# janisgp/go_with_the_flows

Measured on AMD Instinct MI355X. Metric: point-flow fwd+logdet Mpoints/sec (B x 2048 pts), higher is better.
Workload: dtype f32 (split-f16 x3 MFMA, fp32 accumulate); 1 GPU; configs[1] airplane generative (config_generative_modeling_airplane.yaml): K=4 flows x 33 couplings, f=37, G=128, B=64 x N=2048, inverse + sum(logvars) + mixture NLL, eval BN -- leads the line because it is the largest single-GPU config of BASELINE.json (configs[1]); the north-star shape B=32 x 2048, f=64 is also.m1; per_gpu_batch=64, components=4, couplings_per_component=33, f=37, G=128, direction=inverse, point_definition=one 3-D point through one component stack (coords + sum logvars)

## Files before the change

go_with_the_flows_amd/csrc/gwtf_film.hip:

```cpp
#include <hip/hip_runtime.h>
#include "gwtf_layout.h"
#include "../../include/gwtf.h"

namespace {

constexpr int kBTe = 16;

typedef float f32x4 __attribute__((ext_vector_type(4)));

template <int MB, int kGCH>
__global__ __launch_bounds__(MB > 4 ? 512 : 256) void film_eval_kernel(const float* __restrict__ g, const float* __restrict__ pf,
                                                        float* __restrict__ out, int B, int G, int C, int f, float eps) {
  constexpr int FP = 16 * MB;
  __shared__ __align__(16) float hb[2][16][FP + 4];
  const int c = blockIdx.x, br = blockIdx.y, b0 = blockIdx.z * kBTe;
  const int lane = threadIdx.x & 63, wave = threadIdx.x >> 6;
  const int q = lane >> 4, i16 = lane & 15;
  const GwtfPackF P(FP, G);
  const int GP = P.GP();
  const float* w = pf + ((size_t)c * 2 + br) * P.branch_size();
  const size_t FS = gwtf_film_out_size(FP);
  const bool own = wave < MB;
  const int ft = 16 * wave + i16;
  const int brow = b0 + i16;
  const float* grow = g + (size_t)(brow < B ? brow : B - 1) * G;
  const float* l0 = w + P.l0t(0) + 4 * ft;
  const float* l1 = w + P.l0t(1) + 4 * ft;
  const bool gvec = (G & 3) == 0;

  f32x4 acc[2] = {{0.f, 0.f, 0.f, 0.f}, {0.f, 0.f, 0.f, 0.f}};
  f32x4 w1[2][MB];
  if (own) {
#pragma unroll
    for (int kg = 0; kg < MB; ++kg)
#pragma unroll
      for (int which = 0; which < 2; ++which)
#pragma unroll
        for (int t = 0; t < 4; ++t) w1[which][kg][t] = w[P.l1t(which) + ((size_t)(4 * kg + q) * FP + ft) * 4 + t];
    for (int i0 = 0; i0 < GP; i0 += kGCH) {
      f32x4 a4[kGCH / 16], b4[2][kGCH / 16];
#pragma unroll
      for (int kg = 0; kg < kGCH / 16; ++kg) {
        if (i0 + 16 * kg < GP) {
          const int col = i0 + 16 * kg + 4 * q;
          if (gvec) {
            a4[kg] = *reinterpret_cast<const f32x4*>(grow + (col < G ? col : G - 4));
          } else {
#pragma unroll
            for (int t = 0; t < 4; ++t) a4[kg][t] = grow[col + t < G ? col + t : G - 1];
          }
          b4[0][kg] = *reinterpret_cast<const f32x4*>(l0 + (size_t)col * FP);
          b4[1][kg] = *reinterpret_cast<const f32x4*>(l1 + (size_t)col * FP);
        }
      }
#pragma unroll
      for (int kg = 0; kg < kGCH / 16; ++kg) {
        if (i0 + 16 * kg < GP) {
#pragma unroll
          for (int t = 0; t < 4; ++t) {
            acc[0] = __builtin_amdgcn_mfma_f32_16x16x4f32(a4[kg][t], b4[0][kg][t], acc[0], 0, 0, 0);
            acc[1] = __builtin_amdgcn_mfma_f32_16x16x4f32(a4[kg][t], b4[1][kg][t], acc[1], 0, 0, 0);
          }
        }
      }
    }
#pragma unroll
    for (int which = 0; which < 2; ++which) {
      const float sc = w[P.s(which) + ft], sh = w[P.t(which) + ft];
#pragma unroll
      for (int r = 0; r < 4; ++r) {
        const float h = fmaf(acc[which][r], sc, sh);
        hb[which][4 * q + r][ft] = h / (1.0f + expf(-h));
      }
    }
  }
  __syncthreads();
  if (!own) return;
  f32x4 o[2];
#pragma unroll
  for (int which = 0; which < 2; ++which) {
    const float bias = w[P.l1b(which) + ft];
    o[which] = f32x4{bias, bias, bias, bias};
  }
#pragma unroll
  for (int kg = 0; kg < MB; ++kg) {
    const f32x4 a0 = *reinterpret_cast<const f32x4*>(&hb[0][i16][16 * kg + 4 * q]);
    const f32x4 a1 = *reinterpret_cast<const f32x4*>(&hb[1][i16][16 * kg + 4 * q]);
#pragma unroll
    for (int t = 0; t < 4; ++t) {
      o[0] = __builtin_amdgcn_mfma_f32_16x16x4f32(a0[t], w1[0][kg][t], o[0], 0, 0, 0);
      o[1] = __builtin_amdgcn_mfma_f32_16x16x4f32(a1[t], w1[1][kg][t], o[1], 0, 0, 0);
    }
  }
  const float c1 = w[P.c1() + ft], w20 = w[P.w2() + ft], w21 = w[P.w2() + FP + ft];
  const float qnan = __builtin_bit_cast(float, 0x7fc00000u);
  const float poison = w[P.poison()];
#pragma unroll
  for (int r = 0; r < 4; ++r) {
    const int b = b0 + 4 * q + r;
    if (b < B) {
      float cv = 0.f, u0 = 0.f, u1 = 0.f;
      if (ft < f) {
        const float a = eps + expf(o[0][r]);
        cv = c1 + o[1][r] / a;
        u0 = w20 * a;
        u1 = w21 * a;
        if (gwtf_nonfinite(o[0][r]) || gwtf_nonfinite(o[1][r])) cv = u0 = u1 = qnan;
      }
      float* ob = out + ((size_t)b * C + c) * FS + (size_t)br * 3 * FP + ft;
      ob[0] = cv;
      ob[FP] = u0;
      ob[2 * FP] = u1;
      if (ft < 2) out[((size_t)b * C + c) * FS + 6 * FP + 2 * br + ft] = w[P.b2() + ft] + poison;
    }
  }
}

}

extern "C" int gwtf_film_forward(const float* g, const float* packed_film, float* film_out, int B, int G, int C, int f, float eps,
                                 void* stream) {
  if (B <= 0 || G <= 0 || C <= 0 || f <= 0 || f > GWTF_MAX_FP || !g || !packed_film || !film_out) return GWTF_E_BADARG;
  const int FP = gwtf_padded_width(f);
  hipStream_t st = (hipStream_t)stream;
  const dim3 grid(C, 2, (B + kBTe - 1) / kBTe);
  const bool many = (long)grid.x * grid.y * grid.z > 768;
#define GWTF_FILM_EVAL(MB_)                                                                                                  \
  if (many) hipLaunchKernelGGL((film_eval_kernel<MB_, 64>), grid, dim3(MB_ > 4 ? 512 : 256), 0, st, g, packed_film, film_out, B, G, C, f, eps); \
  else hipLaunchKernelGGL((film_eval_kernel<MB_, 128>), grid, dim3(MB_ > 4 ? 512 : 256), 0, st, g, packed_film, film_out, B, G, C, f, eps)
  switch (FP / 16) {
    case 1: GWTF_FILM_EVAL(1); break;
    case 2: GWTF_FILM_EVAL(2); break;
    case 3: GWTF_FILM_EVAL(3); break;
    case 4: GWTF_FILM_EVAL(4); break;
    case 5: GWTF_FILM_EVAL(5); break;
    case 6: GWTF_FILM_EVAL(6); break;
    case 7: GWTF_FILM_EVAL(7); break;
    default: GWTF_FILM_EVAL(8); break;
  }
#undef GWTF_FILM_EVAL
  return (int)hipGetLastError();
}
```

go_with_the_flows_amd/csrc/gwtf_nll.hip:

```cpp
#include <hip/hip_runtime.h>
#include <math.h>
#include "../../include/gwtf.h"

namespace {

constexpr int kMaxK = 64;
constexpr int kThreads = 256;
constexpr int kPtsPerBlock = 512;

__global__ __launch_bounds__(1024) void nll_kernel(const float* __restrict__ z, const float* __restrict__ logdet,
                                                       const float* __restrict__ mu0, const float* __restrict__ lv0,
                                                       const float* __restrict__ logits, float* __restrict__ point_lse,
                                                       float* __restrict__ nll_shape, int K, int B, int N) {
  __shared__ float s_logw[kMaxK];
  __shared__ float s_mu[kMaxK][3], s_lv[kMaxK][3], s_iv[kMaxK][3];
  __shared__ float s_part[16];
  const int b = blockIdx.y;
  const int ppb = gridDim.x == 1 ? N : kPtsPerBlock;
  if (threadIdx.x < 64) {
    float m = -INFINITY;
    for (int k = 0; k < K; ++k) m = fmaxf(m, logits[(size_t)b * K + k]);
    float s = 0.f;
    for (int k = 0; k < K; ++k) s += expf(logits[(size_t)b * K + k] - m);
    const float lse = m + logf(s);
    for (int k = threadIdx.x; k < K; k += 64) s_logw[k] = logf(expf(logits[(size_t)b * K + k])) - lse;
  }
  for (int t = threadIdx.x; t < K * 3; t += blockDim.x) {
    const int k = t / 3, d = t % 3;
    const float l = lv0[((size_t)k * B + b) * 3 + d];
    s_mu[k][d] = mu0[((size_t)k * B + b) * 3 + d];
    s_lv[k][d] = l;
    s_iv[k][d] = 1.0f / expf(l);
  }
  __syncthreads();
  const float half_log2pi3 = 0.5f * 3.0f * 1.8378770664093453f;
  float local = 0.f;
  const int n_end = min(N, (int)(blockIdx.x + 1) * ppb);
  for (int n = blockIdx.x * ppb + threadIdx.x; n < n_end; n += blockDim.x) {
    float m = -INFINITY, s = 0.f;
    bool nan_seen = false;
    for (int k = 0; k < K; ++k) {
      float qsum = 0.f;
#pragma unroll
      for (int d = 0; d < 3; ++d) {
        const size_t o = (((size_t)k * B + b) * 3 + d) * N + n;
        const float diff = z[o] - s_mu[k][d];
        qsum += (s_lv[k][d] + logdet[o]) + diff * diff * s_iv[k][d];
      }
      float lp = -0.5f * qsum - half_log2pi3 + s_logw[k];
      asm volatile("" : "+v"(lp));
      nan_seen |= (__float_as_uint(lp) & 0x7fffffffu) > 0x7f800000u;
      if (lp == -INFINITY) continue;
      if (lp > m || k == 0) {
        s = s * expf(m - lp) + 1.0f;
        m = lp;
      } else {
        s += expf(lp - m);
      }
    }
    const float lse = nan_seen ? __uint_as_float(0x7fc00000u) : m + logf(s);
    if (point_lse) point_lse[(size_t)b * N + n] = lse;
    local += lse;
  }
#pragma unroll
  for (int off = 32; off > 0; off >>= 1) local += __shfl_down(local, off);
  if ((threadIdx.x & 63) == 0) s_part[threadIdx.x >> 6] = local;
  __syncthreads();
  if (threadIdx.x == 0) {
    float t = 0.f;
    for (int w = 0; w < (int)blockDim.x / 64; ++w) t += s_part[w];
    if (gridDim.x == 1) nll_shape[b] = -t;
    else atomicAdd(&nll_shape[b], -t);
  }
}

__global__ __launch_bounds__(kThreads) void nll_bwd_kernel(const float* __restrict__ z, const float* __restrict__ logdet,
                                                           const float* __restrict__ mu0, const float* __restrict__ lv0,
                                                           const float* __restrict__ logits,
                                                           const float* __restrict__ point_lse,
                                                           const float* __restrict__ g_nll, float* __restrict__ g_z,
                                                           float* __restrict__ g_ld, float* __restrict__ g_mu0,
                                                           float* __restrict__ g_lv0, float* __restrict__ g_logits, int K,
                                                           int B, int N) {
  __shared__ float s_logw[kMaxK], s_sm[kMaxK];
  __shared__ float s_mu[kMaxK][3], s_lv[kMaxK][3], s_iv[kMaxK][3];
  __shared__ float s_acc[kMaxK][7];
  const int b = blockIdx.y;
  if (threadIdx.x < 64) {
    float m = -INFINITY;
    for (int k = 0; k < K; ++k) m = fmaxf(m, logits[(size_t)b * K + k]);
    float sden = 0.f;
    for (int k = 0; k < K; ++k) sden += expf(logits[(size_t)b * K + k] - m);
    const float lse = m + logf(sden);
    for (int k = threadIdx.x; k < K; k += 64) {
      s_logw[k] = logf(expf(logits[(size_t)b * K + k])) - lse;
      s_sm[k] = expf(logits[(size_t)b * K + k] - lse);
    }
  }
  for (int t = threadIdx.x; t < K * 3; t += blockDim.x) {
    const int k = t / 3, d = t % 3;
    const float l = lv0[((size_t)k * B + b) * 3 + d];
    s_mu[k][d] = mu0[((size_t)k * B + b) * 3 + d];
    s_lv[k][d] = l;
    s_iv[k][d] = 1.0f / expf(l);
  }
  for (int t = threadIdx.x; t < K * 7; t += blockDim.x) (&s_acc[0][0])[t] = 0.f;
  __syncthreads();
  const float half_log2pi3 = 0.5f * 3.0f * 1.8378770664093453f;
  const float gb = g_nll[b];
  const int n_end = min(N, (int)(blockIdx.x + 1) * kPtsPerBlock);
  for (int k = 0; k < K; ++k) {
    float a[7] = {0.f, 0.f, 0.f, 0.f, 0.f, 0.f, 0.f};
    for (int n = blockIdx.x * kPtsPerBlock + threadIdx.x; n < n_end; n += blockDim.x) {
      float diff[3], qsum = 0.f;
#pragma unroll
      for (int d = 0; d < 3; ++d) {
        const size_t o = (((size_t)k * B + b) * 3 + d) * N + n;
        diff[d] = z[o] - s_mu[k][d];
        qsum += (s_lv[k][d] + logdet[o]) + diff[d] * diff[d] * s_iv[k][d];
      }
      const float r = expf(-0.5f * qsum - half_log2pi3 + s_logw[k] - point_lse[(size_t)b * N + n]) * gb;
#pragma unroll
      for (int d = 0; d < 3; ++d) {
        const size_t o = (((size_t)k * B + b) * 3 + d) * N + n;
        const float w = diff[d] * s_iv[k][d];
        g_z[o] = r * w;
        g_ld[o] = 0.5f * r;
        a[d] -= r * w;
        a[3 + d] += r * (0.5f - 0.5f * diff[d] * w);
      }
      a[6] += r;
    }
#pragma unroll
    for (int i = 0; i < 7; ++i) {
#pragma unroll
      for (int off = 32; off > 0; off >>= 1) a[i] += __shfl_down(a[i], off);
    }
    if ((threadIdx.x & 63) == 0) {
#pragma unroll
      for (int i = 0; i < 7; ++i) atomicAdd(&s_acc[k][i], a[i]);
    }
  }
  __syncthreads();
  for (int t = threadIdx.x; t < K * 7; t += blockDim.x) {
    const int k = t / 7, i = t % 7;
    const float v = s_acc[k][i];
    if (i < 3) atomicAdd(&g_mu0[((size_t)k * B + b) * 3 + i], v);
    else if (i < 6) atomicAdd(&g_lv0[((size_t)k * B + b) * 3 + (i - 3)], v);
    else {
      const int pts = n_end - blockIdx.x * kPtsPerBlock;
      atomicAdd(&g_logits[(size_t)b * K + k], -v + gb * (float)pts * s_sm[k]);
    }
  }
}

}

extern "C" int gwtf_mixture_nll_backward(const float* z, const float* logdet, const float* mu0, const float* lv0,
                                         const float* logits, const float* point_lse, const float* g_nll, float* g_z,
                                         float* g_logdet, float* g_mu0, float* g_lv0, float* g_logits, int K, int B, int N,
                                         void* stream) {
  if (K <= 0 || K > kMaxK || B <= 0 || N <= 0 || !z || !logdet || !mu0 || !lv0 || !logits || !point_lse || !g_nll || !g_z ||
      !g_logdet || !g_mu0 || !g_lv0 || !g_logits)
    return GWTF_E_BADARG;
  hipStream_t st = (hipStream_t)stream;
  hipError_t e = hipMemsetAsync(g_mu0, 0, sizeof(float) * (size_t)K * B * 3, st);
  if (e == hipSuccess) e = hipMemsetAsync(g_lv0, 0, sizeof(float) * (size_t)K * B * 3, st);
  if (e == hipSuccess) e = hipMemsetAsync(g_logits, 0, sizeof(float) * (size_t)B * K, st);
  if (e != hipSuccess) return (int)e;
  const dim3 grid((N + kPtsPerBlock - 1) / kPtsPerBlock, B);
  hipLaunchKernelGGL(nll_bwd_kernel, grid, dim3(kThreads), 0, st, z, logdet, mu0, lv0, logits, point_lse, g_nll, g_z,
                     g_logdet, g_mu0, g_lv0, g_logits, K, B, N);
  return (int)hipGetLastError();
}

extern "C" int gwtf_mixture_nll(const float* z, const float* logdet, const float* mu0, const float* lv0,
                                const float* logits, float* point_lse, float* nll_shape, int K, int B, int N,
                                void* stream) {
  if (K <= 0 || K > kMaxK || B <= 0 || N <= 0 || !z || !logdet || !mu0 || !lv0 || !logits || !nll_shape)
    return GWTF_E_BADARG;
  hipStream_t st = (hipStream_t)stream;
  if (N <= 4096 && B >= 16) {
    hipLaunchKernelGGL(nll_kernel, dim3(1, B), dim3(1024), 0, st, z, logdet, mu0, lv0, logits, point_lse, nll_shape, K, B, N);
    return (int)hipGetLastError();
  }
  hipError_t e = hipMemsetAsync(nll_shape, 0, sizeof(float) * (size_t)B, st);
  if (e != hipSuccess) return (int)e;
  const dim3 grid((N + kPtsPerBlock - 1) / kPtsPerBlock, B);
  hipLaunchKernelGGL(nll_kernel, grid, dim3(kThreads), 0, st, z, logdet, mu0, lv0, logits, point_lse, nll_shape, K, B, N);
  return (int)hipGetLastError();
}
```

Baseline: 1076 Mpoints/s.

## Software-pipeline FiLM GEMM loads and batch mixture NLL loads across components

The FiLM kernel gains a fast path, used when G is a multiple of 4 and GP divides the chunk size. It prefetches the next chunk of g and layer-0 weights while issuing MFMAs on the current chunk, and parameter loads are hoisted ahead of the GEMM. Launches now use 64*MB threads, which drops the idle waves that previously existed for small MB. The NLL kernel issues the first group of component loads before the shared-memory setup and the __syncthreads. It then processes two points per thread, loading four components at a time to raise memory-level parallelism. The cost is higher register pressure and more complex control flow.

```diff
diff --git a/go_with_the_flows_amd/csrc/gwtf_film.hip b/go_with_the_flows_amd/csrc/gwtf_film.hip
--- a/go_with_the_flows_amd/csrc/gwtf_film.hip
+++ b/go_with_the_flows_amd/csrc/gwtf_film.hip
@@ -8,10 +8,29 @@
 
 typedef float f32x4 __attribute__((ext_vector_type(4)));
 
-template <int MB, int kGCH>
+template <int NKG>
+struct FilmChunk {
+  f32x4 a[NKG], b[2][NKG];
+  __device__ __forceinline__ void load(int kg, const float* grow, const float* l0, const float* l1, int i0, int q, int G, int FP) {
+    const int col = i0 + 16 * kg + 4 * q;
+    a[kg] = *reinterpret_cast<const f32x4*>(grow + (col < G ? col : G - 4));
+    b[0][kg] = *reinterpret_cast<const f32x4*>(l0 + (size_t)col * FP);
+    b[1][kg] = *reinterpret_cast<const f32x4*>(l1 + (size_t)col * FP);
+  }
+  __device__ __forceinline__ void mfma(int kg, f32x4 (&acc)[2]) const {
+#pragma unroll
+    for (int t = 0; t < 4; ++t) {
+      acc[0] = __builtin_amdgcn_mfma_f32_16x16x4f32(a[kg][t], b[0][kg][t], acc[0], 0, 0, 0);
+      acc[1] = __builtin_amdgcn_mfma_f32_16x16x4f32(a[kg][t], b[1][kg][t], acc[1], 0, 0, 0);
+    }
+  }
+};
+
+template <int MB, int kGCH, bool kFast>
 __global__ __launch_bounds__(MB > 4 ? 512 : 256) void film_eval_kernel(const float* __restrict__ g, const float* __restrict__ pf,
                                                         float* __restrict__ out, int B, int G, int C, int f, float eps) {
   constexpr int FP = 16 * MB;
+  constexpr int NKG = kGCH / 16;
   __shared__ __align__(16) float hb[2][16][FP + 4];
   const int c = blockIdx.x, br = blockIdx.y, b0 = blockIdx.z * kBTe;
   const int lane = threadIdx.x & 63, wave = threadIdx.x >> 6;
@@ -20,68 +39,84 @@
   const int GP = P.GP();
   const float* w = pf + ((size_t)c * 2 + br) * P.branch_size();
   const size_t FS = gwtf_film_out_size(FP);
-  const bool own = wave < MB;
   const int ft = 16 * wave + i16;
   const int brow = b0 + i16;
   const float* grow = g + (size_t)(brow < B ? brow : B - 1) * G;
   const float* l0 = w + P.l0t(0) + 4 * ft;
   const float* l1 = w + P.l0t(1) + 4 * ft;
-  const bool gvec = (G & 3) == 0;
 
   f32x4 acc[2] = {{0.f, 0.f, 0.f, 0.f}, {0.f, 0.f, 0.f, 0.f}};
   f32x4 w1[2][MB];
-  if (own) {
+  float sc[2], sh[2], bias[2], c1, w20, w21, poison, b2v;
+  FilmChunk<NKG> ch;
+  if constexpr (kFast) {
 #pragma unroll
-    for (int kg = 0; kg < MB; ++kg)
+    for (int kg = 0; kg < NKG; ++kg) ch.load(kg, grow, l0, l1, 0, q, G, FP);
+  }
 #pragma unroll
-      for (int which = 0; which < 2; ++which)
+  for (int kg = 0; kg < MB; ++kg)
 #pragma unroll
-        for (int t = 0; t < 4; ++t) w1[which][kg][t] = w[P.l1t(which) + ((size_t)(4 * kg + q) * FP + ft) * 4 + t];
+    for (int which = 0; which < 2; ++which)
+#pragma unroll
+      for (int t = 0; t < 4; ++t) w1[which][kg][t] = w[P.l1t(which) + ((size_t)(4 * kg + q) * FP + ft) * 4 + t];
+#pragma unroll
+  for (int which = 0; which < 2; ++which) {
+    sc[which] = w[P.s(which) + ft];
+    sh[which] = w[P.t(which) + ft];
+    bias[which] = w[P.l1b(which) + ft];
+  }
+  c1 = w[P.c1() + ft];
+  w20 = w[P.w2() + ft];
+  w21 = w[P.w2() + FP + ft];
+  poison = w[P.poison()];
+  b2v = w[P.b2() + (ft & 1)];
+  if constexpr (kFast) {
+    int i0 = 0;
+    for (; i0 + kGCH < GP; i0 += kGCH) {
+#pragma unroll
+      for (int kg = 0; kg < NKG; ++kg) {
+        ch.mfma(kg, acc);
+        ch.load(kg, grow, l0, l1, i0 + kGCH, q, G, FP);
+        __builtin_amdgcn_sched_barrier(0);
+      }
+    }
+#pragma unroll
+    for (int kg = 0; kg < NKG; ++kg) ch.mfma(kg, acc);
+  } else {
+    const bool gvec = (G & 3) == 0;
     for (int i0 = 0; i0 < GP; i0 += kGCH) {
-      f32x4 a4[kGCH / 16], b4[2][kGCH / 16];
 #pragma unroll
-      for (int kg = 0; kg < kGCH / 16; ++kg) {
+      for (int kg = 0; kg < NKG; ++kg) {
         if (i0 + 16 * kg < GP) {
-          const int col = i0 + 16 * kg + 4 * q;
           if (gvec) {
-            a4[kg] = *reinterpret_cast<const f32x4*>(grow + (col < G ? col : G - 4));
+            ch.load(kg, grow, l0, l1, i0, q, G, FP);
           } else {
+            const int col = i0 + 16 * kg + 4 * q;
 #pragma unroll
-            for (int t = 0; t < 4; ++t) a4[kg][t] = grow[col + t < G ? col + t : G - 1];
+            for (int t = 0; t < 4; ++t) ch.a[kg][t] = grow[col + t < G ? col + t : G - 1];
+            ch.b[0][kg] = *reinterpret_cast<const f32x4*>(l0 + (size_t)col * FP);
+            ch.b[1][kg] = *reinterpret_cast<const f32x4*>(l1 + (size_t)col * FP);
           }
-          b4[0][kg] = *reinterpret_cast<const f32x4*>(l0 + (size_t)col * FP);
-          b4[1][kg] = *reinterpret_cast<const f32x4*>(l1 + (size_t)col * FP);
         }
       }
 #pragma unroll
-      for (int kg = 0; kg < kGCH / 16; ++kg) {
-        if (i0 + 16 * kg < GP) {
-#pragma unroll
-          for (int t = 0; t < 4; ++t) {
-            acc[0] = __builtin_amdgcn_mfma_f32_16x16x4f32(a4[kg][t], b4[0][kg][t], acc[0], 0, 0, 0);
-            acc[1] = __builtin_amdgcn_mfma_f32_16x16x4f32(a4[kg][t], b4[1][kg][t], acc[1], 0, 0, 0);
-          }
-        }
-      }
-    }
-#pragma unroll
-    for (int which = 0; which < 2; ++which) {
-      const float sc = w[P.s(which) + ft], sh = w[P.t(which) + ft];
-#pragma unroll
-      for (int r = 0; r < 4; ++r) {
-        const float h = fmaf(acc[which][r], sc, sh);
-        hb[which][4 * q + r][ft] = h / (1.0f + expf(-h));
+      for (int kg = 0; kg < NKG; ++kg) {
+        if (i0 + 16 * kg < GP) ch.mfma(kg, acc);
       }
     }
   }
+#pragma unroll
+  for (int which = 0; which < 2; ++which) {
+#pragma unroll
+    for (int r = 0; r < 4; ++r) {
+      const float h = fmaf(acc[which][r], sc[which], sh[which]);
+      hb[which][4 * q + r][ft] = h / (1.0f + expf(-h));
+    }
+  }
   __syncthreads();
-  if (!own) return;
   f32x4 o[2];
 #pragma unroll
-  for (int which = 0; which < 2; ++which) {
-    const float bias = w[P.l1b(which) + ft];
-    o[which] = f32x4{bias, bias, bias, bias};
-  }
+  for (int which = 0; which < 2; ++which) o[which] = f32x4{bias[which], bias[which], bias[which], bias[which]};
 #pragma unroll
   for (int kg = 0; kg < MB; ++kg) {
     const f32x4 a0 = *reinterpret_cast<const f32x4*>(&hb[0][i16][16 * kg + 4 * q]);
@@ -92,9 +127,8 @@
       o[1] = __builtin_amdgcn_mfma_f32_16x16x4f32(a1[t], w1[1][kg][t], o[1], 0, 0, 0);
     }
   }
-  const float c1 = w[P.c1() + ft], w20 = w[P.w2() + ft], w21 = w[P.w2() + FP + ft];
   const float qnan = __builtin_bit_cast(float, 0x7fc00000u);
-  const float poison = w[P.poison()];
+  const float b2p = b2v + poison;
 #pragma unroll
   for (int r = 0; r < 4; ++r) {
     const int b = b0 + 4 * q + r;
@@ -111,7 +145,7 @@
       ob[0] = cv;
       ob[FP] = u0;
       ob[2 * FP] = u1;
-      if (ft < 2) out[((size_t)b * C + c) * FS + 6 * FP + 2 * br + ft] = w[P.b2() + ft] + poison;
+      if (ft < 2) out[((size_t)b * C + c) * FS + 6 * FP + 2 * br + ft] = b2p;
     }
   }
 }
@@ -125,9 +159,18 @@
   hipStream_t st = (hipStream_t)stream;
   const dim3 grid(C, 2, (B + kBTe - 1) / kBTe);
   const bool many = (long)grid.x * grid.y * grid.z > 768;
-#define GWTF_FILM_EVAL(MB_)                                                                                                  \
-  if (many) hipLaunchKernelGGL((film_eval_kernel<MB_, 64>), grid, dim3(MB_ > 4 ? 512 : 256), 0, st, g, packed_film, film_out, B, G, C, f, eps); \
-  else hipLaunchKernelGGL((film_eval_kernel<MB_, 128>), grid, dim3(MB_ > 4 ? 512 : 256), 0, st, g, packed_film, film_out, B, G, C, f, eps)
+  const int GP = GwtfPackF(FP, G).GP();
+  const bool fast64 = (G & 3) == 0 && GP % 64 == 0, fast128 = (G & 3) == 0 && GP % 128 == 0;
+#define GWTF_FILM_EVAL_(MB_, CH_, FAST_)                                                                                        \
+  hipLaunchKernelGGL((film_eval_kernel<MB_, CH_, FAST_>), grid, dim3(64 * MB_), 0, st, g, packed_film, film_out, B, G, C, f, eps)
+#define GWTF_FILM_EVAL(MB_)                                                                                                    \
+  if (many) {                                                                                                                  \
+    if (fast64) GWTF_FILM_EVAL_(MB_, 64, true);                                                                                \
+    else GWTF_FILM_EVAL_(MB_, 64, false);                                                                                      \
+  } else {                                                                                                                     \
+    if (fast128) GWTF_FILM_EVAL_(MB_, 128, true);                                                                              \
+    else GWTF_FILM_EVAL_(MB_, 128, false);                                                                                     \
+  }
   switch (FP / 16) {
     case 1: GWTF_FILM_EVAL(1); break;
     case 2: GWTF_FILM_EVAL(2); break;
@@ -139,5 +182,6 @@
     default: GWTF_FILM_EVAL(8); break;
   }
 #undef GWTF_FILM_EVAL
+#undef GWTF_FILM_EVAL_
   return (int)hipGetLastError();
 }
diff --git a/go_with_the_flows_amd/csrc/gwtf_nll.hip b/go_with_the_flows_amd/csrc/gwtf_nll.hip
--- a/go_with_the_flows_amd/csrc/gwtf_nll.hip
+++ b/go_with_the_flows_amd/csrc/gwtf_nll.hip
@@ -7,6 +7,61 @@
 constexpr int kMaxK = 64;
 constexpr int kThreads = 256;
 constexpr int kPtsPerBlock = 512;
+
+constexpr int kPass = 2;
+
+struct NllPoint {
+  float m, s;
+  bool nan_seen;
+};
+
+template <int NB>
+__device__ __forceinline__ void nll_load(const float* __restrict__ z, const float* __restrict__ logdet, int kb, int B, int b, int N,
+                                         const unsigned (&np)[kPass], float (&zz)[kPass][4][3], float (&ld)[kPass][4][3]) {
+  asm volatile("" : "+s"(kb));
+#pragma unroll
+  for (int j = 0; j < NB; ++j)
+#pragma unroll
+    for (int d = 0; d < 3; ++d) {
+      const size_t row = (((size_t)(kb + j) * B + b) * 3 + d) * N;
+#pragma unroll
+      for (int p = 0; p < kPass; ++p) {
+        zz[p][j][d] = (z + row)[np[p]];
+        ld[p][j][d] = (logdet + row)[np[p]];
+      }
+    }
+  __builtin_amdgcn_sched_barrier(0);
+}
+
+template <int NB>
+__device__ __forceinline__ void nll_accumulate(const float (*s_mu)[3], const float (*s_lv)[3], const float (*s_iv)[3], const float* s_logw,
+                                               int kb, const float (&zz)[kPass][4][3], const float (&ld)[kPass][4][3],
+                                               NllPoint (&pt)[kPass]) {
+  const float half_log2pi3 = 0.5f * 3.0f * 1.8378770664093453f;
+#pragma unroll
+  for (int p = 0; p < kPass; ++p)
+#pragma unroll
+    for (int j = 0; j < NB; ++j) {
+      const int k = kb + j;
+      float qsum = 0.f;
+#pragma unroll
+      for (int d = 0; d < 3; ++d) {
+        const float diff = zz[p][j][d] - s_mu[k][d];
+        qsum += (s_lv[k][d] + ld[p][j][d]) + diff * diff * s_iv[k][d];
+      }
+      float lp = -0.5f * qsum - half_log2pi3 + s_logw[k];
+      asm volatile("" : "+v"(lp));
+      pt[p].nan_seen |= (__float_as_uint(lp) & 0x7fffffffu) > 0x7f800000u;
+      if (!(lp == -INFINITY)) {
+        if (lp > pt[p].m || k == 0) {
+          pt[p].s = pt[p].s * expf(pt[p].m - lp) + 1.0f;
+          pt[p].m = lp;
+        } else {
+          pt[p].s += expf(lp - pt[p].m);
+        }
+      }
+    }
+}
 
 __global__ __launch_bounds__(1024) void nll_kernel(const float* __restrict__ z, const float* __restrict__ logdet,
                                                        const float* __restrict__ mu0, const float* __restrict__ lv0,
@@ -17,6 +72,19 @@
   __shared__ float s_part[16];
   const int b = blockIdx.y;
   const int ppb = gridDim.x == 1 ? N : kPtsPerBlock;
+  const int n_end = min(N, (int)(blockIdx.x + 1) * ppb);
+  const int n_first = blockIdx.x * ppb + threadIdx.x;
+  unsigned np[kPass];
+  float zz[kPass][4][3], ld[kPass][4][3];
+  bool ahead = K >= 4;
+  if (ahead) {
+#pragma unroll
+    for (int p = 0; p < kPass; ++p) {
+      const int n = n_first + p * (int)blockDim.x;
+      np[p] = n < n_end ? n : min(n_first, n_end - 1);
+    }
+    nll_load<4>(z, logdet, 0, B, b, N, np, zz, ld);
+  }
   if (threadIdx.x < 64) {
     float m = -INFINITY;
     for (int k = 0; k < K; ++k) m = fmaxf(m, logits[(size_t)b * K + k]);
@@ -33,34 +101,44 @@
     s_iv[k][d] = 1.0f / expf(l);
   }
   __syncthreads();
-  const float half_log2pi3 = 0.5f * 3.0f * 1.8378770664093453f;
   float local = 0.f;
-  const int n_end = min(N, (int)(blockIdx.x + 1) * ppb);
-  for (int n = blockIdx.x * ppb + threadIdx.x; n < n_end; n += blockDim.x) {
-    float m = -INFINITY, s = 0.f;
-    bool nan_seen = false;
-    for (int k = 0; k < K; ++k) {
-      float qsum = 0.f;
-#pragma unroll
-      for (int d = 0; d < 3; ++d) {
-        const size_t o = (((size_t)k * B + b) * 3 + d) * N + n;
-        const float diff = z[o] - s_mu[k][d];
-        qsum += (s_lv[k][d] + logdet[o]) + diff * diff * s_iv[k][d];
-      }
-      float lp = -0.5f * qsum - half_log2pi3 + s_logw[k];
-      asm volatile("" : "+v"(lp));
-      nan_seen |= (__float_as_uint(lp) & 0x7fffffffu) > 0x7f800000u;
-      if (lp == -INFINITY) continue;
-      if (lp > m || k == 0) {
-        s = s * expf(m - lp) + 1.0f;
-        m = lp;
-      } else {
-        s += expf(lp - m);
-      }
-    }
-    const float lse = nan_seen ? __uint_as_float(0x7fc00000u) : m + logf(s);
-    if (point_lse) point_lse[(size_t)b * N + n] = lse;
-    local += lse;
+  for (int n0 = n_first; n0 < n_end; n0 += kPass * blockDim.x) {
+    NllPoint pt[kPass];
+#pragma unroll
+    for (int p = 0; p < kPass; ++p) {
+      const int n = n0 + p * (int)blockDim.x;
+      np[p] = n < n_end ? n : n0;
+      pt[p] = NllPoint{-INFINITY, 0.f, false};
+    }
+    int kb = 0;
+    if (ahead) {
+      nll_accumulate<4>(s_mu, s_lv, s_iv, s_logw, 0, zz, ld, pt);
+      kb = 4;
+      ahead = false;
+    }
+#pragma unroll 1
+    for (; kb + 4 <= K; kb += 4) {
+      nll_load<4>(z, logdet, kb, B, b, N, np, zz, ld);
+      nll_accumulate<4>(s_mu, s_lv, s_iv, s_logw, kb, zz, ld, pt);
+    }
+#define GWTF_NLL_REST(NB_)                                      \
+  nll_load<NB_>(z, logdet, kb, B, b, N, np, zz, ld);            \
+  nll_accumulate<NB_>(s_mu, s_lv, s_iv, s_logw, kb, zz, ld, pt)
+    switch (K - kb) {
+      case 3: GWTF_NLL_REST(3); break;
+      case 2: GWTF_NLL_REST(2); break;
+      case 1: GWTF_NLL_REST(1); break;
+      default: break;
+    }
+#undef GWTF_NLL_REST
+#pragma unroll
+    for (int p = 0; p < kPass; ++p) {
+      if (n0 + p * (int)blockDim.x < n_end) {
+        const float lse = pt[p].nan_seen ? __uint_as_float(0x7fc00000u) : pt[p].m + logf(pt[p].s);
+        if (point_lse) point_lse[(size_t)b * N + np[p]] = lse;
+        local += lse;
+      }
+    }
   }
 #pragma unroll
   for (int off = 32; off > 0; off >>= 1) local += __shfl_down(local, off);
```

Result: no change. 1083 Mpoints/s, median of 6 (+0.7%).
